# inai17ibar/video-diffusion-pipeline-parallel

Measured on AMD Instinct MI355X. Metric: steady-state videos/sec (whole node), SVD 14f x 25step, higher is better.
Workload: dtype f16

## Files before the change

### video-diffusion-pipeline-parallel_amd/csrc/gemm.hip

```cpp
#include <cstring>
#include "gemm_args.h"
#include <stdlib.h>

using namespace spgemm;

namespace {


template <int BM, int BN, int WM, int WN, int STAGES>
__global__ __launch_bounds__(WM *WN * 64, 2) void gemm_f16_kernel(const GemmArgs p) {
  constexpr int NW = WM * WN;
  constexpr int THREADS = NW * 64;
  constexpr int WTM = BM / WM, WTN = BN / WN;
  constexpr int TN = WTN / 16;
  constexpr int TM = WTM / 16;
  constexpr int A_BYTES = BM * BK * 2;
  constexpr int B_BYTES = BN * BK * 2;
  constexpr int STAGE = A_BYTES + B_BYTES;
  constexpr int A_LOADS = BM / 8 / NW;
  constexpr int B_LOADS = BN / 8 / NW;
  constexpr int L = A_LOADS + B_LOADS;
  static_assert(A_LOADS * 8 * NW == BM && B_LOADS * 8 * NW == BN, "tile rows must split evenly over waves");
  static_assert(STAGES == 2 || STAGES == 3, "2- or 3-deep ring");
  extern __shared__ __attribute__((aligned(16))) char smem[];
// ... 505 lines not shown
    const int bms[2] = {256, 192}, bns[2] = {256, 320};
    for (int bi = 0; bi < 2; ++bi)
      for (int ni = 0; ni < 2; ++ni) {
        if ((bns[ni] == 256 && !ok256) || (bns[ni] == 320 && !ok320)) continue;
        const int blocks = ((d->m + bms[bi] - 1) / bms[bi]) * (d->n / bns[ni]);
        double score = (double)blocks / (((blocks + 255) / 256) * 256.0);
        if (bms[bi] == 192) score -= 0.06;
        if (bns[ni] == 320) score -= 0.01;
        if (score > best) { best = score; bm = bms[bi]; bn = bns[ni]; }
      }
    if (route == 2) {
      if ((g_route_bn == 256 && ok256) || (g_route_bn == 320 && ok320)) bn = g_route_bn;
      if (g_route_bm == 192 || g_route_bm == 256 || (g_route_bm == 128 && bn == 256)) bm = g_route_bm;
    }
    return launch_pp(a, bm, bn, s);
  }
  if (n128 && d->m >= 4096) return launch<256, 128, 4, 2, 3>(a, s);
  if (n128) return launch<128, 128, 2, 2, 2>(a, s);
  if (d->n % 160 == 0) return launch<128, 160, 2, 2, 2>(a, s);
  return launch<128, 64, 2, 2, 2>(a, s);
}

}

namespace spgemm {
static thread_local char g_last_kernel[96] = "";
void note_kernel(const char *fmt, ...) {
  va_list ap;
  va_start(ap, fmt);
  vsnprintf(g_last_kernel, sizeof(g_last_kernel), fmt, ap);
  va_end(ap);
}
void note_kernel_suffix(const char *suffix) {
  const size_t have = strlen(g_last_kernel);
  snprintf(g_last_kernel + have, sizeof(g_last_kernel) - have, "%s", suffix);
}
}

extern "C" const char *sp_gemm_last_kernel(void) { return spgemm::g_last_kernel; }

extern "C" size_t sp_gemm_workspace_bytes(const sp_gemm_desc *d) {
  if (!d || d->m <= 0 || d->n <= 0 || d->cin <= 0) return 0;
  const int taps = d->mode == SP_A_CONV3X3 ? 9 : d->mode == SP_A_TEMPORAL3 ? 3 : 1;
  int sk = splitk_slices(d, taps, false);
  const int forced = splitk_slices(d, taps, true);
  if (forced > sk) sk = forced;
  size_t need = (size_t)sk * d->m * d->n * sizeof(float);
  const int ltiles = d->n % 320 == 0 ? d->n / 320 : d->n / 256;
  const size_t ln_part = (d->ln_out && ltiles > 1) ? (size_t)d->m * ltiles * 2 * sizeof(float) : 0;
  return need > ln_part ? need : ln_part;
}

extern "C" int sp_gemm_set_route(int route, int bm, int bn) {
  SP_REQUIRE(route >= 0 && route <= 4,
             "sp_gemm_set_route: route %d (0 auto, 1 small tiles, 2 ping-pong, 3 persistent-stream, 4 split-K)", route);
  SP_REQUIRE(bm == 0 || bm == 128 || bm == 192 || bm == 256, "sp_gemm_set_route: bm %d", bm);
  SP_REQUIRE(bn == 0 || bn == 256 || bn == 320 || bn == 192, "sp_gemm_set_route: bn %d", bn);
  g_route = route; g_route_bm = bm; g_route_bn = bn;
  return SP_OK;
}

extern "C" int sp_gemm_f32out_f16(const void *a_, int64_t lda, const void *w, void *d, int m, int n, int k,
                                  const void *zero_page, void *stream) {
  SP_REQUIRE(a_ && w && d && zero_page, "sp_gemm_f32out_f16: null a/w/d/zero_page");
  SP_REQUIRE(m > 0 && n > 0 && n % 256 == 0, "sp_gemm_f32out_f16: n=%d must be a positive multiple of 256 (m=%d)", n, m);
  SP_REQUIRE(k >= 64 && k % 64 == 0, "sp_gemm_f32out_f16: k=%d must be a multiple of 64", k);
  SP_REQUIRE(lda >= k && lda % 8 == 0, "sp_gemm_f32out_f16: lda=%lld invalid", (long long)lda);
  SP_REQUIRE(((uintptr_t)d & 15) == 0, "sp_gemm_f32out_f16: d must be 16-byte aligned");
  GemmArgs a{};
  a.a = (const f16 *)a_; a.w = (const f16 *)w; a.zero = (const char *)zero_page;
  a.lda = lda; a.mode = SP_A_LINEAR; a.cin = k; a.taps = 1; a.m = m; a.n = n; a.k = k;
  a.oscale = 1.0f; a.bias2_rows = m; a.ldb2 = n;
  a.ksplit = 1; a.partial = (float *)d;
  return spgemm::launch_pp(a, 256, 256, (hipStream_t)stream);
}

extern "C" int sp_gemm_f16(const sp_gemm_desc *d, void *stream) {
  SP_REQUIRE(d != nullptr, "sp_gemm_f16: null descriptor");
  SP_REQUIRE(d->a && d->w && d->d && d->zero_page, "sp_gemm_f16: null a/w/d/zero_page");
  SP_REQUIRE(d->m > 0 && d->n > 0, "sp_gemm_f16: m,n must be positive (m=%d n=%d)", d->m, d->n);
  SP_REQUIRE(d->cin > 0 && d->cin % 64 == 0, "sp_gemm_f16: cin=%d must be a multiple of 64", d->cin);
  SP_REQUIRE(d->n % 64 == 0, "sp_gemm_f16: n=%d must be a multiple of 64", d->n);
  SP_REQUIRE(d->mode >= SP_A_LINEAR && d->mode <= SP_A_TEMPORAL3, "sp_gemm_f16: bad mode %d", d->mode);
  SP_REQUIRE(d->lda >= d->cin && d->lda % 8 == 0, "sp_gemm_f16: lda=%lld invalid", (long long)d->lda);
  SP_REQUIRE(d->ldd % 8 == 0 || d->n_store > 0, "sp_gemm_f16: ldd must be a multiple of 8");
  GemmArgs a{};
#ifdef SP_GEMM_EXPERIMENTS
  { const char *e = getenv("SP_GEMM_DBG"); a.dbg = e ? atoi(e) : 0; }
  { const char *e = getenv("SP_GEMM_STAGGER"); a.stagger = e ? atoi(e) : 0; }
#endif
  a.a = (const f16 *)d->a; a.w = (const f16 *)d->w; a.bias = d->bias; a.bias2 = d->bias2;
  a.res1 = (const f16 *)d->res1; a.res2 = (const f16 *)d->res2; a.d = (f16 *)d->d;
  a.ln_stats = d->ln_stats; a.ln_colsum = d->ln_colsum;
  a.ln_out = d->ln_out; a.ln_out_eps = d->ln_out_eps;
  a.gn_part = nullptr;
  if (d->gn_part) {
    SP_REQUIRE(!d->geglu && !d->ln_stats && !d->ln_out && !d->euler_out && d->n_store == 0 &&
                   d->m % 256 == 0 && (d->n % 256 == 0 || d->n % 320 == 0) && ((uintptr_t)d->gn_part & 15) == 0,
               "sp_gemm_f16: gn_part needs whole 256-row tiles (m = %d), n a multiple of 256 or 320 (n = %d), no geglu / "
               "folded LayerNorm / ln_out / n_store / Euler tail, and a 16-byte aligned buffer", d->m, d->n);
    a.gn_part = d->gn_part;
  }
  a.w_group_rows = 0; a.w_group_stride = 0;
  if (d->w_group_rows != 0) {
    SP_REQUIRE(d->w_group_rows > 0 && d->w_group_rows % 128 == 0 && d->w_group_stride > 0 && d->w_group_stride % 8 == 0 &&
                   d->mode == SP_A_LINEAR && !d->geglu && !d->euler_out && (d->n % 256 == 0 || d->n % 320 == 0) &&
                   !d->ln_stats && !d->ln_colsum,
               "sp_gemm_f16: per-row-group weights need SP_A_LINEAR, no geglu / Euler tail / folded LayerNorm (ln_stats), n a "
               "multiple of 256 or 320, w_group_rows a positive multiple of 128 (got %lld) and w_group_stride a positive multiple "
               "of 8 (got %lld)", (long long)d->w_group_rows, (long long)d->w_group_stride);
    a.w_group_rows = d->w_group_rows; a.w_group_stride = d->w_group_stride;
// ... 78 lines not shown
```

### video-diffusion-pipeline-parallel_amd/csrc/gemm_args.h

```cpp
#pragma once
#include "common.h"

namespace spgemm {

constexpr int BK = 64;

template <int N>
__device__ __forceinline__ void wait_vm_lgkm() {
  asm volatile("s_waitcnt vmcnt(%0) lgkmcnt(0)" ::"n"(N) : "memory");
}

struct GemmArgs {
  const f16 *a;
  const f16 *a2;
  int64_t lda2;
  int cin2;
  const f16 *w;
  const float *bias;
  const float *bias2;
  const f16 *res1;
  const f16 *res2;
  const f16 *eul_lat; f16 *eul_out; const f16 *eul_u; const float *eul_gs;
  int64_t eul_ldu, eul_hw;
  int eul_frames;
  float eul_c_out, eul_c_skip, eul_inv_sigma, eul_dt;
  const float *ln_stats;
  const float *ln_colsum;
  float *ln_out;
  float ln_out_eps;
  float *gn_part;
  float *ln_part;
  f16 *d;
  const char *zero;
  int64_t lda, ldr1, ldr2, ldd, hw, bias2_rows, ldb2;
  int64_t w_group_rows, w_group_stride;
  int mode, cin, taps;
  int n_img, hin, win, hout, wout, stride, ups;
  int frames;
  int m, n, k;
  float oscale, r1scale, r2scale;
  int geglu, n_store;
  int tiles_m, tiles_n;
  int ksplit;
  float *partial;
  int dbg;
  int stagger;
};

__device__ __forceinline__ int xcd_remap(int bid, int nwg) {
  const int q = nwg >> 3, r = nwg & 7;
  const int xcd = bid & 7;
  const int base = xcd < r ? xcd * (q + 1) : r * (q + 1) + (xcd - r) * q;
  return base + (bid >> 3);
}


void note_kernel(const char *fmt, ...);
void note_kernel_suffix(const char *suffix);

int launch_pp(GemmArgs &a, int bm, int bn, hipStream_t s);

bool ps_supported(const GemmArgs &a, int bm, int bn);
int launch_ps(GemmArgs &a, int bm, int bn, hipStream_t s);

}
```

### video-diffusion-pipeline-parallel_amd/csrc/gemm_pp.hip

```cpp
#include "gemm_args.h"
#include <stdlib.h>
#include <type_traits>

namespace spgemm {
namespace {

constexpr int PBK = 32, PNW = 8;


#ifdef SP_GEMM_EXPERIMENTS
constexpr int PP_TRACE_WGS = 16384, PP_TRACE_SLOTS = 12;
__device__ long long g_pp_trace[PP_TRACE_WGS * PP_TRACE_SLOTS];
#define PP_TRACE(slot)                                                                              \
  do {                                                                                              \
    if (threadIdx.x == 0 && blockIdx.x < PP_TRACE_WGS)                                              \
      g_pp_trace[blockIdx.x * PP_TRACE_SLOTS + (slot)] = wall_clock64();                            \
  } while (0)
#define PP_TRACE_CLK(slot)                                                                          \
  do {                                                                                              \
    if (threadIdx.x == 0 && blockIdx.x < PP_TRACE_WGS)                                              \
      g_pp_trace[blockIdx.x * PP_TRACE_SLOTS + (slot)] = (long long)__builtin_amdgcn_s_memtime();   \
  } while (0)
#else
#define PP_TRACE(slot) do {} while (0)
#define PP_TRACE_CLK(slot) do {} while (0)
#endif

__device__ __forceinline__ int swz4(int row) { return (0x78 >> (((row >> 2) & 3) * 2)) & 3; }

#ifndef SP_PP_STAGES_192_256
#define SP_PP_STAGES_192_256 4
#endif
constexpr int pp_stages(int bm, int bn) { return bm == 128 ? 3 : (bm == 192 && bn == 256 ? SP_PP_STAGES_192_256 : 4); }

template <int N>
__device__ __forceinline__ void wait_vm() { asm volatile("s_waitcnt vmcnt(%0)" ::"n"(N) : "memory"); }

template <int L>
__device__ __forceinline__ void wait_dma(int ksteps_left) {
  if (ksteps_left >= 3) wait_vm<3 * L>();
  else if (ksteps_left == 2) wait_vm<2 * L>();
  else if (ksteps_left == 1) wait_vm<L>();
  else wait_vm<0>();
}

#define WROWS_OF(pbm, wtm) ((pbm) / (wtm))
template <int PBM, int BN, int TN, int TM, int WTN, int WTM, bool GEGLU, int NT, bool GNRES = false>
__device__ __forceinline__ void pp_epilogue(const GemmArgs &p, f32x4 (&acc)[TN][TM], char *smem, int tile_m,
                                            int tile_n, int wm, int wn, int tid, int fr, int fq) {
  constexpr int bno = GEGLU ? BN / 2 : BN;
  constexpr int cpr = bno >> 3;
  constexpr int TNO = GEGLU ? TN / 2 : TN;
  constexpr int NCH = PBM * cpr, ITERS = (NCH + NT - 1) / NT, ITERS_A = ITERS / 2;
  static_assert(cpr % 8 == 0, "chunk swizzle works on aligned groups of 8 chunks");
  const int ncols_total = GEGLU ? p.n / 2 : p.n;
  const int nstore = p.n_store > 0 ? p.n_store : ncols_total;
  const int64_t mbase = (int64_t)tile_m * PBM;

  auto res_src = [&](const f16 *res, int64_t ldr, int it) -> const f16 * {
    const int idx = tid + it * NT;
    const int r = idx / cpr, c = idx - r * cpr;
    const int64_t m = mbase + r;
    const int col = tile_n * bno + c * 8;
    const bool ok = idx < NCH && m < p.m && col + 8 <= nstore;
    return ok ? res + m * ldr + col : (const f16 *)p.zero;
  };

  if (p.ln_stats) {
    f32x2 st[TM];
    const __amdgpu_buffer_rsrc_t s_rsrc = __builtin_amdgcn_make_buffer_rsrc(
        (void *)p.ln_stats, 0, (int)min((int64_t)p.m * 8, (int64_t)0x7fffffff), 0x00020000);
#pragma unroll
    for (int j = 0; j < TM; ++j)
      st[j] = __builtin_bit_cast(f32x2, __builtin_amdgcn_raw_buffer_load_b64(
          s_rsrc, (int)((mbase + wm * WTM + j * 16 + fr) * 8), 0, 0));
#pragma unroll
    for (int i = 0; i < TN; ++i) {
      const int n = tile_n * BN + wn * WTN + i * 16 + 4 * fq;
      const f32x4 cs = *(const f32x4 *)(p.ln_colsum + n);
      f32x4 b = {0.f, 0.f, 0.f, 0.f};
      if (p.bias) b = *(const f32x4 *)(p.bias + n);
#pragma unroll
      for (int j = 0; j < TM; ++j) acc[i][j] = (acc[i][j] - st[j][0] * cs) * st[j][1] + b;
      __builtin_amdgcn_sched_barrier(0);
    }
  }
  if constexpr (!GEGLU) {
    if (p.gn_part && !p.res1 && !p.res2) {
      auto row16_sum = [](float v) {
        v += __builtin_bit_cast(float, __builtin_amdgcn_mov_dpp(__builtin_bit_cast(int, v), 0xB1, 0xF, 0xF, true));
        v += __builtin_bit_cast(float, __builtin_amdgcn_mov_dpp(__builtin_bit_cast(int, v), 0x4E, 0xF, 0xF, true));
        v += __builtin_bit_cast(float, __builtin_amdgcn_mov_dpp(__builtin_bit_cast(int, v), 0x141, 0xF, 0xF, true));
        v += __builtin_bit_cast(float, __builtin_amdgcn_mov_dpp(__builtin_bit_cast(int, v), 0x140, 0xF, 0xF, true));
        return v;
      };
      float *dst = p.gn_part + (((int64_t)tile_m * WROWS_OF(PBM, WTM) + wm) * p.n + (int64_t)tile_n * BN + wn * WTN) * 2;
#pragma unroll
      for (int i = 0; i < TN; ++i) {
        f32x4 sm = {0.f, 0.f, 0.f, 0.f}, sq = {0.f, 0.f, 0.f, 0.f};
#pragma unroll
        for (int j = 0; j < TM; ++j) {
          const f32x4 v = acc[i][j] * p.oscale;
          sm += v;
          sq += v * v;
        }
#pragma unroll
        for (int r = 0; r < 4; ++r) { sm[r] = row16_sum(sm[r]); sq[r] = row16_sum(sq[r]); }
        if (fr == 0) {
          float *o = dst + (i * 16 + 4 * fq) * 2;
          *(f32x4 *)o = (f32x4){sm[0], sq[0], sm[1], sq[1]};
          *(f32x4 *)(o + 4) = (f32x4){sm[2], sq[2], sm[3], sq[3]};
        }
      }
    }
  }
  f16x8 q1[ITERS];
  if (p.res1) {
#pragma unroll
    for (int it = 0; it < ITERS_A; ++it) q1[it] = *(const f16x8 *)res_src(p.res1, p.ldr1, it);
  }
  PP_TRACE(4);

#pragma unroll
  for (int i = 0; i < TNO; ++i) {
    const int col = (GEGLU ? (wn * WTN) / 2 : wn * WTN) + i * 16 + 4 * fq;
#pragma unroll
    for (int j = 0; j < TM; ++j) {
      f16x4 o;
      if constexpr (!GEGLU) {
        const f32x4 v = acc[i][j] * p.oscale;
        o = (f16x4){(f16)v[0], (f16)v[1], (f16)v[2], (f16)v[3]};
      } else {
        const f32x4 h = acc[2 * i][j] * p.oscale, g = acc[2 * i + 1][j];
        const f32x2 ga = gelu2_f((f32x2){g[0], g[1]}), gb = gelu2_f((f32x2){g[2], g[3]});
        o = (f16x4){(f16)(h[0] * ga[0]), (f16)(h[1] * ga[1]), (f16)(h[2] * gb[0]), (f16)(h[3] * gb[1])};
      }
      const int row = wm * WTM + j * 16 + fr;
      *(f16x4 *)(smem + row * (bno * 2) + ((((col >> 3) ^ (fr & 7))) << 4) + (col & 4) * 2) = o;
    }
  }
  if (p.res1) {
#pragma unroll
    for (int it = ITERS_A; it < ITERS; ++it) q1[it] = *(const f16x8 *)res_src(p.res1, p.ldr1, it);
  }
  asm volatile("s_waitcnt lgkmcnt(0)\n\ts_barrier" ::: "memory");
  PP_TRACE(6);

  f16x8 o[ITERS];
#pragma unroll
  for (int it = 0; it < ITERS; ++it) {
    const int idx = tid + it * NT;
    const int r = idx / cpr, c = idx - r * cpr;
    o[it] = *(const f16x8 *)(smem + r * (bno * 2) + ((c ^ (r & 7)) << 4));
  }
  const bool gn_res = GNRES && !GEGLU && PBM == 256 && p.gn_part && (p.res1 || p.res2);
  if (gn_res) asm volatile("s_waitcnt lgkmcnt(0)\n\ts_barrier" ::: "memory");
  if (p.res1 || p.res2) {
// ... 107 lines not shown
#pragma unroll
        for (int e = 0; e < 4; ++e) { pt[(grp * Q + quad) * 8 + 2 * e] = sm[e]; pt[(grp * Q + quad) * 8 + 2 * e + 1] = sq[e]; }
      }
      asm volatile("s_waitcnt lgkmcnt(0)\n\ts_barrier" ::: "memory");
      if (tid < 2 * Q) {
        const int half = tid / Q, qd = tid - half * Q;
        f32x4 a = {0.f, 0.f, 0.f, 0.f}, b = {0.f, 0.f, 0.f, 0.f};
        for (int sub = 0; sub < RG; ++sub) {
          const float *src = pt + ((half * RG + sub) * Q + qd) * 8;
          a += *(const f32x4 *)src; b += *(const f32x4 *)(src + 4);
        }
        float *dst = p.gn_part + (((int64_t)tile_m * 2 + half) * p.n + (int64_t)tile_n * bno + qd * 4) * 2;
        *(f32x4 *)dst = a;
        *(f32x4 *)(dst + 4) = b;
      }
    }
  }
}

#ifdef SP_GEMM_EXPERIMENTS
template <int TN, int TM, int NAP, int NBP, int NWV>
__device__ __forceinline__ void mfma_block(f32x4 (&acc)[TN][TM], const f16x8 (&fw)[TN], const f16x8 (&fa)[TM],
                                           const f16 *(&aptr)[NAP], int (&astep)[NAP], const f16 *(&bptr)[NBP],
                                           char *dsa, char *dsb, int pieces) {
  constexpr int NP = NAP + NBP, NM = TN * TM, GAP = NM / (NP + 1);
#pragma unroll
  for (int i = 0; i < TN; ++i) {
#pragma unroll
    for (int j = 0; j < TM; ++j) {
      acc[i][j] = __builtin_amdgcn_mfma_f32_16x16x32_f16(fw[i], fa[j], acc[i][j], 0, 0, 0);
      const int q1 = i * TM + j + 1;
      if (q1 % GAP == 0 && q1 / GAP <= NP) {
        const int pc = q1 / GAP - 1;
        if (pieces & (1 << pc)) {
          if (pc < NAP) {
            glds16(aptr[pc], dsa + pc * (NWV * 1024));
            aptr[pc] += astep[pc];
          } else {
            glds16(bptr[pc - NAP], dsb + (pc - NAP) * (NWV * 1024));
            bptr[pc - NAP] += PBK;
          }
        }
      }
    }
  }
}
#endif

template <int BM, int BN, int EXP>
__global__ __launch_bounds__(BM == 128 ? 256 : 512, 2) void gemm_pp_kernel(const GemmArgs p) {
  constexpr int PBM = BM;
  constexpr bool SPLITK = (EXP & 128) != 0;
  constexpr bool A2 = (EXP & 4096) != 0;
  constexpr int NWV = BM == 128 ? 4 : 8, NT = NWV * 64, WROWS = NWV / 4;
  constexpr int PSTAGES = pp_stages(BM, BN), PDIST = PSTAGES - 1;
  constexpr int TN = BN / 4 / 16;
  constexpr int TM = BM / WROWS / 16;
  constexpr int WTN = BN / 4, WTM = BM / WROWS;
  constexpr int A_BYTES = PBM * 64, B_BYTES = BN * 64, STAGE = A_BYTES + B_BYTES;
  constexpr int A_PIECES = BM / 16, B_PIECES = BN / 16;
  constexpr int A_LOADS = (A_PIECES + NWV - 1) / NWV, A_LOADS_HI = A_PIECES / NWV;
  constexpr int A_SPLIT = A_PIECES % NWV == 0 ? NWV : A_PIECES % NWV;
  constexpr int B_LOADS_LO = (B_PIECES + NWV - 1) / NWV;
  constexpr int B_LOADS_HI = B_PIECES / NWV;
  constexpr int B_SPLIT = B_PIECES % NWV == 0 ? NWV : B_PIECES % NWV;
  static_assert((B_SPLIT == NWV || B_SPLIT == 4) && (A_SPLIT == NWV || A_SPLIT == 4), "wave halves must have uniform DMA counts");
#ifdef SP_GEMM_EXPERIMENTS
  constexpr bool HALO_COUNT = (EXP & 16) != 0;
  constexpr int L_EARLY = (HALO_COUNT ? 0 : A_LOADS) + B_LOADS_LO;
  constexpr int L_LATE = (HALO_COUNT ? 0 : (A_SPLIT == NWV ? A_LOADS : A_LOADS_HI)) + (B_SPLIT == NWV ? B_LOADS_LO : B_LOADS_HI);
#else
  constexpr int L_EARLY = A_LOADS + B_LOADS_LO;
  constexpr int L_LATE = (A_SPLIT == NWV ? A_LOADS : A_LOADS_HI) + (B_SPLIT == NWV ? B_LOADS_LO : B_LOADS_HI);
#endif
  extern __shared__ __attribute__((aligned(16))) char smem[];

  const int tid = threadIdx.x, lane = tid & 63;
  const int wave = __builtin_amdgcn_readfirstlane(tid >> 6);
  const int wm = wave >> 2, wn = wave & 3;
  const bool late = NWV == 8 && wave >= 4;
#ifdef SP_GEMM_EXPERIMENTS
  if (p.stagger > 0 && blockIdx.x < 256) {
    const int d = ((blockIdx.x >> 3) & 3) * p.stagger;
    for (int i = 0; i < d; ++i) __builtin_amdgcn_s_sleep(30);
  }
#endif
  PP_TRACE(0);
#ifdef SP_GEMM_EXPERIMENTS
  if (tid == 0 && blockIdx.x < PP_TRACE_WGS) {
    const unsigned hw = __builtin_amdgcn_s_getreg((31 << 11) | 4);
    const unsigned xcc = __builtin_amdgcn_s_getreg((31 << 11) | 20);
    g_pp_trace[blockIdx.x * PP_TRACE_SLOTS + 5] = ((long long)xcc << 32) | hw;
  }
#endif

  constexpr int GM = BM == 128 ? 8 : 4;
  const int nwg = p.tiles_m * p.tiles_n;
  int bid = blockIdx.x, kslice = 0;
  if constexpr (SPLITK) { kslice = bid / nwg; bid -= kslice * nwg; }
  const int t = xcd_remap(bid, nwg);
  const int per_group = GM * p.tiles_n;
  const int group = t / per_group;
  const int first_m = group * GM;
  const int gsz = min(p.tiles_m - first_m, GM);
  const int in_group = t - group * per_group;
  const int tile_n = in_group / gsz;
// ... 76 lines not shown
  };

  const f16 *bptr[B_LOADS_LO];
#pragma unroll
  for (int j = 0; j < B_LOADS_LO; ++j) {
    const int piece = j * NWV + wave;
    const int r = piece * 16 + lrow;
    const int n = tile_n * BN + (r < BN ? r : 0);
    bptr[j] = p.w + (int64_t)n * p.k + (lchunk ^ swz4(r)) * 8;
    if (p.w_group_rows > 0) bptr[j] += ((int64_t)tile_m * PBM / p.w_group_rows) * p.w_group_stride;
  }

  bool skip_a = false;
  auto stage = [&](int slot) {
    char *sa = smem + slot * STAGE;
    char *sb = sa + A_BYTES;
#pragma unroll
    for (int i = 0; i < A_LOADS; ++i) {
      if ((i < A_LOADS_HI || wave < A_SPLIT) && !skip_a) {
        glds16(aptr[i], sa + (i * NWV + wave) * 1024);
        aptr[i] += astep[i];
      }
    }
#pragma unroll
    for (int j = 0; j < B_LOADS_LO; ++j) {
      if (j < B_LOADS_HI || wave < B_SPLIT) {
        glds16(bptr[j], sb + (j * NWV + wave) * 1024);
        bptr[j] += PBK;
      }
    }
  };

  f32x4 acc[TN][TM], bias_v[TN];
#pragma unroll
  for (int i = 0; i < TN; ++i) {
    bias_v[i] = (f32x4){0.f, 0.f, 0.f, 0.f};
    if (p.bias && !p.ln_stats && !SPLITK)
      bias_v[i] = *(const f32x4 *)(p.bias + tile_n * BN + wn * WTN + i * 16 + 4 * (lane >> 4));
  }
  __builtin_amdgcn_sched_barrier(0);

  int nk = p.k >> 5, kbeg = 0;
  if constexpr (SPLITK) {
    kbeg = (int)((int64_t)kslice * nk / p.ksplit);
    nk = (int)((int64_t)(kslice + 1) * nk / p.ksplit) - kbeg;
  }
  const int fr = lane & 15, fq = lane >> 4;
  const int rd_chunk = (fq ^ swz4(fr)) << 4;
  int offw[TN], offa[TM];
#pragma unroll
  for (int i = 0; i < TN; ++i) offw[i] = (wn * WTN + i * 16 + fr) * 64 + rd_chunk;
#pragma unroll
  for (int j = 0; j < TM; ++j) offa[j] = (wm * WTM + j * 16 + fr) * 64 + rd_chunk;

  int staged = 0, in_tap = 0, tap = 0, stage_slot = 0, read_slot = 0;
  auto stage_next = [&]() {
    if (in_tap == cpt && (!A2 || tap < p.taps)) { ++tap; in_tap = 0; set_tap(tap); }
#ifdef SP_GEMM_EXPERIMENTS
    if constexpr ((EXP & 16) != 0) skip_a = tap > 0;
#endif
    stage(stage_slot);
    stage_slot = stage_slot + 1 == PSTAGES ? 0 : stage_slot + 1;
    ++staged; ++in_tap;
  };
  tap = kbeg / cpt;
  in_tap = kbeg - tap * cpt;
  set_tap(tap);
  if (kbeg) {
#pragma unroll
    for (int i = 0; i < A_LOADS; ++i) aptr[i] += in_tap * astep[i];
#pragma unroll
    for (int j = 0; j < B_LOADS_LO; ++j) bptr[j] += (int64_t)kbeg * PBK;
  }
  PP_TRACE(10);
#pragma unroll
  for (int s = 0; s < PDIST; ++s)
    if (s < nk) stage_next();
  PP_TRACE(11);
  __builtin_amdgcn_sched_barrier(0);
  if (p.bias2 && !SPLITK) {
    int brow[TM];
#pragma unroll
    for (int j = 0; j < TM; ++j) {
      const int m = tile_m * PBM + wm * WTM + j * 16 + fr;
      brow[j] = m < p.m ? m / (int)p.bias2_rows : 0;
    }
#pragma unroll
    for (int i = 0; i < TN; ++i) {
      const int n = tile_n * BN + wn * WTN + i * 16 + 4 * fq;
#pragma unroll
      for (int j = 0; j < TM; ++j) acc[i][j] = *(const f32x4 *)(p.bias2 + (int64_t)brow[j] * p.ldb2 + n) + bias_v[i];
      __builtin_amdgcn_sched_barrier(0);
    }
  } else {
#pragma unroll
    for (int i = 0; i < TN; ++i)
#pragma unroll
      for (int j = 0; j < TM; ++j) acc[i][j] = bias_v[i];
  }
  {
    const int left = min(PDIST - 1, nk - 1);
    if (late) wait_dma<L_LATE>(left); else wait_dma<L_EARLY>(left);
  }
  __builtin_amdgcn_s_barrier();
  if (late) __builtin_amdgcn_s_barrier();
  PP_TRACE(1);
  PP_TRACE_CLK(8);

#ifdef SP_GEMM_EXPERIMENTS
  constexpr int dbg = EXP;
  constexpr bool DMA_IN_COMPUTE = (dbg & 4) != 0;
#endif
  for (int kt = 0; kt < nk; ++kt) {
    const bool issue = kt + PDIST < nk;
    const char *sa = smem + read_slot * STAGE;
    read_slot = read_slot + 1 == PSTAGES ? 0 : read_slot + 1;
    const char *sb = sa + A_BYTES;
    f16x8 fw[TN], fa[TM];
#ifdef SP_GEMM_EXPERIMENTS
    if ((dbg & 64) && kt > 0) {
#pragma unroll
      for (int i = 0; i < TN; ++i) fw[i] = (f16x8){1, 2, 3, 4, 5, 6, 7, (f16)kt};
#pragma unroll
      for (int j = 0; j < TM; ++j) fa[j] = (f16x8){1, 2, 3, 4, 5, 6, 7, (f16)lane};
    } else
#endif
    {
#pragma unroll
      for (int i = 0; i < TN; ++i) fw[i] = *(const f16x8 *)(sb + offw[i]);
#pragma unroll
      for (int j = 0; j < TM; ++j) fa[j] = *(const f16x8 *)(sa + offa[j]);
    }
#ifdef SP_GEMM_EXPERIMENTS
    if constexpr ((dbg & 32) != 0) {
      const f16x2 sc2 = {(f16)(1.0f + 0.001f * lane), (f16)1.0f}, sh2 = {(f16)0.01f, (f16)(0.002f * lane)};
#pragma unroll
      for (int j = 0; j < TM; ++j) {
#pragma unroll
        for (int e = 0; e < 4; ++e) {
          f16x2 v = {fa[j][2 * e], fa[j][2 * e + 1]};
          v = __builtin_elementwise_fma(v, sc2, sh2);
          const f16x2 t = __builtin_elementwise_exp2(v * (f16x2){(f16)-1.4427f, (f16)-1.4427f}) + (f16x2){(f16)1.0f, (f16)1.0f};
          v = v * (f16x2){(f16)__builtin_amdgcn_rcph(t[0]), (f16)__builtin_amdgcn_rcph(t[1])};
          fa[j][2 * e] = v[0]; fa[j][2 * e + 1] = v[1];
        }
      }
    }
#endif
    __builtin_amdgcn_sched_barrier(0);
#ifdef SP_GEMM_EXPERIMENTS
    if constexpr (DMA_IN_COMPUTE) {
      if (issue && in_tap == cpt) { ++tap; in_tap = 0; set_tap(tap); }
      int left = min(PDIST - 2, nk - 2 - kt);
      if (left < 0) left = 0;
      if (late) wait_dma<L_LATE>(left);
    } else
#endif
    {
#ifdef SP_GEMM_EXPERIMENTS
      if constexpr (!(dbg & 1))
#endif
      { if (issue) stage_next(); }
      int left = min(PDIST - 1, nk - 2 - kt);
      if (left < 0) left = 0;
      if (late) wait_dma<L_LATE>(left);
    }
    asm volatile("s_waitcnt lgkmcnt(0)" ::: "memory");
    __builtin_amdgcn_sched_barrier(0);
    __builtin_amdgcn_s_barrier();
    __builtin_amdgcn_sched_barrier(0);
    __builtin_amdgcn_s_setprio(1);
#ifdef SP_GEMM_EXPERIMENTS
    if constexpr (DMA_IN_COMPUTE) {
      char *dsa = smem + stage_slot * STAGE + wave * 1024;
      char *dsb = dsa + A_BYTES;
      int pieces = 0;
      if (issue) {
#pragma unroll
        for (int i = 0; i < A_LOADS; ++i) if (i < A_LOADS_HI || wave < A_SPLIT) pieces |= 1 << i;
#pragma unroll
        for (int j = 0; j < B_LOADS_LO; ++j) if (j < B_LOADS_HI || wave < B_SPLIT) pieces |= 1 << (A_LOADS + j);
      }
      mfma_block<TN, TM, A_LOADS, B_LOADS_LO, NWV>(acc, fw, fa, aptr, astep, bptr, dsa, dsb,
                                              __builtin_amdgcn_readfirstlane(pieces));
      if (issue) {
        stage_slot = stage_slot + 1 == PSTAGES ? 0 : stage_slot + 1;
        ++staged; ++in_tap;
      }
    } else if constexpr ((dbg & 2) != 0) {
#pragma unroll
      for (int i = 0; i < TN; ++i) asm volatile("" ::"v"(fw[i]));
#pragma unroll
      for (int j = 0; j < TM; ++j) asm volatile("" ::"v"(fa[j]));
    } else
#endif
    {
#pragma unroll
      for (int i = 0; i < TN; ++i) {
#pragma unroll
        for (int j = 0; j < TM; ++j)
          acc[i][j] = __builtin_amdgcn_mfma_f32_16x16x32_f16(fw[i], fa[j], acc[i][j], 0, 0, 0);
      }
    }
    __builtin_amdgcn_s_setprio(0);
    if (!late) wait_dma<L_EARLY>(min(PDIST - 1, max(nk - 2 - kt, 0)));
    __builtin_amdgcn_sched_barrier(0);
    __builtin_amdgcn_s_barrier();
    __builtin_amdgcn_sched_barrier(0);
  }
  if (!late) __builtin_amdgcn_s_barrier();
  PP_TRACE_CLK(9);
  PP_TRACE(2);

  if constexpr (SPLITK) {
    float *slab = p.partial + (int64_t)kslice * p.m * p.n;
#pragma unroll
    for (int j = 0; j < TM; ++j) {
      const int64_t m = (int64_t)tile_m * PBM + wm * WTM + j * 16 + fr;
      if (m < p.m) {
#pragma unroll
        for (int i = 0; i < TN; ++i)
          *(f32x4 *)(slab + m * p.n + tile_n * BN + wn * WTN + i * 16 + 4 * fq) = acc[i][j];
      }
    }
  } else if (p.geglu) {
    if constexpr (TN % 2 == 0) pp_epilogue<PBM, BN, TN, TM, WTN, WTM, true, NT>(p, acc, smem, tile_m, tile_n, wm, wn, tid, fr, fq);
  } else {
    pp_epilogue<PBM, BN, TN, TM, WTN, WTM, false, NT, (EXP & 2048) != 0>(p, acc, smem, tile_m, tile_n, wm, wn, tid, fr, fq);
  }
  PP_TRACE(3);
}

template <int BM, int BN, int EXP = 0>
int launch_pp(GemmArgs &a, hipStream_t s) {
  constexpr int NSTG = pp_stages(BM, BN);
  constexpr size_t ring = (size_t)NSTG * (BM + BN) * 64, tile = (size_t)BM * BN * 2;
  constexpr size_t lds = ring > tile ? ring : tile;
  static_assert(lds <= 160 * 1024, "LDS per workgroup");
  static bool attr_set[SP_MAX_DEVICES] = {};
  if (int rc = sp_ensure_dyn_lds((const void *)gemm_pp_kernel<BM, BN, EXP>, (int)lds, attr_set, "sp_gemm_f16(pp)"))
    return rc;
  a.tiles_m = (a.m + BM - 1) / BM;
  a.tiles_n = a.n / BN;
  note_kernel((EXP & 128) ? "gemm_pp_kernel<%d, %d, %d> + splitk_reduce_kernel" : "gemm_pp_kernel<%d, %d, %d>", BM, BN, EXP);
  SP_CLEAR_STALE_ERROR();
  hipLaunchKernelGGL((gemm_pp_kernel<BM, BN, EXP>), dim3(a.tiles_m * a.tiles_n * ((EXP & 128) ? a.ksplit : 1)),
                     dim3(BM == 128 ? 256 : 512), lds, s, a);
  SP_CHECK_LAUNCH("sp_gemm_f16(pp)");
  return SP_OK;
}

}

int launch_pp(GemmArgs &a, int bm, int bn, hipStream_t s) {
  if (a.ksplit >= 1 && a.partial) return launch_pp<256, 256, 128>(a, s);
  if (a.gn_part && (a.res1 || a.res2)) return bn == 256 ? launch_pp<256, 256, 2048>(a, s) : launch_pp<256, 320, 2048>(a, s);
  if (a.a2) return bn == 256 ? launch_pp<256, 256, 4096>(a, s) : launch_pp<256, 320, 4096>(a, s);
#ifdef SP_GEMM_EXPERIMENTS
  if (bm == 256 && bn == 256) switch (a.dbg) {
    case 1: return launch_pp<256, 256, 1>(a, s);
    case 2: return launch_pp<256, 256, 2>(a, s);
    case 3: return launch_pp<256, 256, 3>(a, s);
    case 65: return launch_pp<256, 256, 65>(a, s);
    case 67: return launch_pp<256, 256, 67>(a, s);
    case 4: return launch_pp<256, 256, 4>(a, s);
    default: break;
  }
  if (bm == 256 && bn == 320 && a.dbg == 4) return launch_pp<256, 320, 4>(a, s);
  if (bm == 192 && bn == 256 && a.dbg == 4) return launch_pp<192, 256, 4>(a, s);
  if (a.dbg == 16) {
    if (bm == 256 && bn == 256) return launch_pp<256, 256, 16>(a, s);
    if (bm == 256 && bn == 320) return launch_pp<256, 320, 16>(a, s);
    if (bm == 192 && bn == 256) return launch_pp<192, 256, 16>(a, s);
  }
  if (a.dbg == 32 && bm == 256 && bn == 320) return launch_pp<256, 320, 32>(a, s);
  if (a.dbg == 8) {
    if (bm == 256 && bn == 256) return launch_pp<256, 256, 8>(a, s);
    if (bm == 256 && bn == 320) return launch_pp<256, 320, 8>(a, s);
    if (bm == 192 && bn == 256) return launch_pp<192, 256, 8>(a, s);
  }
#endif
  if (bn == 256) {
    if (bm == 128) return launch_pp<128, 256>(a, s);
    if (bm == 192) return launch_pp<192, 256>(a, s);
    return launch_pp<256, 256>(a, s);
  }
  if (bm == 192) return launch_pp<192, 320>(a, s);
  return launch_pp<256, 320>(a, s);
}

}

#ifdef SP_GEMM_EXPERIMENTS
extern "C" int sp_debug_pp_trace(long long *host, int n_wgs) {
  if (n_wgs > spgemm::PP_TRACE_WGS) n_wgs = spgemm::PP_TRACE_WGS;
  return (int)hipMemcpyFromSymbol(host, HIP_SYMBOL(spgemm::g_pp_trace),
                                  sizeof(long long) * n_wgs * spgemm::PP_TRACE_SLOTS);
}
#endif
```

Baseline: 0.8151.

## Add whole-line paired K-step staging path to ping-pong GEMM

Adds a new ping-pong GEMM mainloop variant that stages two 32-wide K steps at once as full 128-byte lines per row, loaded directly into LDS via buffer/global load-to-LDS instructions, into a two-image double buffer. Out-of-range rows are handled with buffer out-of-bounds offsets instead of zero-page pointers. The variant becomes the default for 256-row tiles when alignment and size checks pass, and a route flag can force the old ring. The aim is wider, better-coalesced loads with fewer barriers and waits per K step. The cost is less pipelining depth (two images instead of a 4-stage ring) and more complex addressing. It also switches the GN sum of squares to explicit fma.

```diff
diff --git a/video-diffusion-pipeline-parallel_amd/csrc/gemm.hip b/video-diffusion-pipeline-parallel_amd/csrc/gemm.hip
--- a/video-diffusion-pipeline-parallel_amd/csrc/gemm.hip
+++ b/video-diffusion-pipeline-parallel_amd/csrc/gemm.hip
@@ -581,11 +581,13 @@
 }
 
 extern "C" int sp_gemm_set_route(int route, int bm, int bn) {
-  SP_REQUIRE(route >= 0 && route <= 4,
-             "sp_gemm_set_route: route %d (0 auto, 1 small tiles, 2 ping-pong, 3 persistent-stream, 4 split-K)", route);
+  SP_REQUIRE(route >= 0 && (route & 15) <= 4 && (route >> 4) <= 2,
+             "sp_gemm_set_route: route %d (0 auto, 1 small tiles, 2 ping-pong, 3 persistent-stream, 4 split-K; "
+             "+16 ping-pong K-step ring only, +32 ping-pong whole-line pairs wherever supported)", route);
   SP_REQUIRE(bm == 0 || bm == 128 || bm == 192 || bm == 256, "sp_gemm_set_route: bm %d", bm);
   SP_REQUIRE(bn == 0 || bn == 256 || bn == 320 || bn == 192, "sp_gemm_set_route: bn %d", bn);
-  g_route = route; g_route_bm = bm; g_route_bn = bn;
+  g_route = route & 15; g_route_bm = bm; g_route_bn = bn;
+  spgemm::g_pp_lines = route >> 4;
   return SP_OK;
 }
 
diff --git a/video-diffusion-pipeline-parallel_amd/csrc/gemm_args.h b/video-diffusion-pipeline-parallel_amd/csrc/gemm_args.h
--- a/video-diffusion-pipeline-parallel_amd/csrc/gemm_args.h
+++ b/video-diffusion-pipeline-parallel_amd/csrc/gemm_args.h
@@ -59,6 +59,7 @@
 void note_kernel_suffix(const char *suffix);
 
 int launch_pp(GemmArgs &a, int bm, int bn, hipStream_t s);
+extern int g_pp_lines;
 
 bool ps_supported(const GemmArgs &a, int bm, int bn);
 int launch_ps(GemmArgs &a, int bm, int bn, hipStream_t s);
diff --git a/video-diffusion-pipeline-parallel_amd/csrc/gemm_pp.hip b/video-diffusion-pipeline-parallel_amd/csrc/gemm_pp.hip
--- a/video-diffusion-pipeline-parallel_amd/csrc/gemm_pp.hip
+++ b/video-diffusion-pipeline-parallel_amd/csrc/gemm_pp.hip
@@ -44,6 +44,23 @@
   else wait_vm<0>();
 }
 
+__device__ __forceinline__ void glds16_s(const char *sbase, unsigned voff, char *lds_dst) {
+  const unsigned l = (unsigned)(uintptr_t)(__attribute__((address_space(3))) char *)lds_dst;
+  asm volatile("s_mov_b32 m0, %2\n\ts_nop 0\n\tglobal_load_lds_dwordx4 %0, %1"
+               :: "v"(voff), "s"(sbase), "s"(l) : "memory", "m0");
+}
+typedef unsigned v4u_t __attribute__((__vector_size__(4 * sizeof(unsigned))));
+constexpr unsigned BUF_OOB = 0x80000000u;
+__device__ __forceinline__ v4u_t buf_rsrc(const void *base) {
+  const uint64_t b = (uint64_t)(uintptr_t)base;
+  return (v4u_t){(unsigned)b, (unsigned)(b >> 32) & 0xffffu, 0x7fffffffu, 0x00020000u};
+}
+__device__ __forceinline__ void blds16(v4u_t rsrc, unsigned voff, unsigned soff, char *lds_dst) {
+  const unsigned l = (unsigned)(uintptr_t)(__attribute__((address_space(3))) char *)lds_dst;
+  asm volatile("s_mov_b32 m0, %3\n\ts_nop 0\n\tbuffer_load_dwordx4 %0, %1, %2 offen lds"
+               :: "v"(voff), "s"(rsrc), "s"(soff), "s"(l) : "memory", "m0");
+}
+
 #define WROWS_OF(pbm, wtm) ((pbm) / (wtm))
 template <int PBM, int BN, int TN, int TM, int WTN, int WTM, bool GEGLU, int NT, bool GNRES = false>
 __device__ __forceinline__ void pp_epilogue(const GemmArgs &p, f32x4 (&acc)[TN][TM], char *smem, int tile_m,
@@ -102,7 +119,8 @@
         for (int j = 0; j < TM; ++j) {
           const f32x4 v = acc[i][j] * p.oscale;
           sm += v;
-          sq += v * v;
+#pragma unroll
+          for (int r = 0; r < 4; ++r) sq[r] = __builtin_fmaf(v[r], v[r], sq[r]);
         }
 #pragma unroll
         for (int r = 0; r < 4; ++r) { sm[r] = row16_sum(sm[r]); sq[r] = row16_sum(sq[r]); }
@@ -316,6 +334,7 @@
   constexpr int PBM = BM;
   constexpr bool SPLITK = (EXP & 128) != 0;
   constexpr bool A2 = (EXP & 4096) != 0;
+  constexpr bool WL = (EXP & 8192) != 0;
   constexpr int NWV = BM == 128 ? 4 : 8, NT = NWV * 64, WROWS = NWV / 4;
   constexpr int PSTAGES = pp_stages(BM, BN), PDIST = PSTAGES - 1;
   constexpr int TN = BN / 4 / 16;
@@ -498,163 +517,295 @@
   for (int i = 0; i < TN; ++i) offw[i] = (wn * WTN + i * 16 + fr) * 64 + rd_chunk;
 #pragma unroll
   for (int j = 0; j < TM; ++j) offa[j] = (wm * WTM + j * 16 + fr) * 64 + rd_chunk;
-
-  int staged = 0, in_tap = 0, tap = 0, stage_slot = 0, read_slot = 0;
-  auto stage_next = [&]() {
-    if (in_tap == cpt && (!A2 || tap < p.taps)) { ++tap; in_tap = 0; set_tap(tap); }
-#ifdef SP_GEMM_EXPERIMENTS
-    if constexpr ((EXP & 16) != 0) skip_a = tap > 0;
-#endif
-    stage(stage_slot);
-    stage_slot = stage_slot + 1 == PSTAGES ? 0 : stage_slot + 1;
-    ++staged; ++in_tap;
+  auto init_acc = [&]() {
+    if (p.bias2 && !SPLITK) {
+      int brow[TM];
+#pragma unroll
+      for (int j = 0; j < TM; ++j) {
+        const int m = tile_m * PBM + wm * WTM + j * 16 + fr;
+        brow[j] = m < p.m ? m / (int)p.bias2_rows : 0;
+      }
+#pragma unroll
+      for (int i = 0; i < TN; ++i) {
+        const int n = tile_n * BN + wn * WTN + i * 16 + 4 * fq;
+#pragma unroll
+        for (int j = 0; j < TM; ++j) acc[i][j] = *(const f32x4 *)(p.bias2 + (int64_t)brow[j] * p.ldb2 + n) + bias_v[i];
+        __builtin_amdgcn_sched_barrier(0);
+      }
+    } else {
+#pragma unroll
+      for (int i = 0; i < TN; ++i)
+#pragma unroll
+        for (int j = 0; j < TM; ++j) acc[i][j] = bias_v[i];
+    }
   };
-  tap = kbeg / cpt;
-  in_tap = kbeg - tap * cpt;
-  set_tap(tap);
-  if (kbeg) {
-#pragma unroll
-    for (int i = 0; i < A_LOADS; ++i) aptr[i] += in_tap * astep[i];
-#pragma unroll
-    for (int j = 0; j < B_LOADS_LO; ++j) bptr[j] += (int64_t)kbeg * PBK;
-  }
-  PP_TRACE(10);
-#pragma unroll
-  for (int s = 0; s < PDIST; ++s)
-    if (s < nk) stage_next();
-  PP_TRACE(11);
-  __builtin_amdgcn_sched_barrier(0);
-  if (p.bias2 && !SPLITK) {
-    int brow[TM];
-#pragma unroll
-    for (int j = 0; j < TM; ++j) {
-      const int m = tile_m * PBM + wm * WTM + j * 16 + fr;
-      brow[j] = m < p.m ? m / (int)p.bias2_rows : 0;
-    }
-#pragma unroll
-    for (int i = 0; i < TN; ++i) {
-      const int n = tile_n * BN + wn * WTN + i * 16 + 4 * fq;
-#pragma unroll
-      for (int j = 0; j < TM; ++j) acc[i][j] = *(const f32x4 *)(p.bias2 + (int64_t)brow[j] * p.ldb2 + n) + bias_v[i];
-      __builtin_amdgcn_sched_barrier(0);
-    }
+
+  if constexpr (!WL) {
+    int staged = 0, in_tap = 0, tap = 0, stage_slot = 0, read_slot = 0;
+    auto stage_next = [&]() {
+      if (in_tap == cpt && (!A2 || tap < p.taps)) { ++tap; in_tap = 0; set_tap(tap); }
+#ifdef SP_GEMM_EXPERIMENTS
+      if constexpr ((EXP & 16) != 0) skip_a = tap > 0;
+#endif
+      stage(stage_slot);
+      stage_slot = stage_slot + 1 == PSTAGES ? 0 : stage_slot + 1;
+      ++staged; ++in_tap;
+    };
+    tap = kbeg / cpt;
+    in_tap = kbeg - tap * cpt;
+    set_tap(tap);
+    if (kbeg) {
+#pragma unroll
+      for (int i = 0; i < A_LOADS; ++i) aptr[i] += in_tap * astep[i];
+#pragma unroll
+      for (int j = 0; j < B_LOADS_LO; ++j) bptr[j] += (int64_t)kbeg * PBK;
+    }
+    PP_TRACE(10);
+#pragma unroll
+    for (int s = 0; s < PDIST; ++s)
+      if (s < nk) stage_next();
+    PP_TRACE(11);
+    __builtin_amdgcn_sched_barrier(0);
+    init_acc();
+    {
+      const int left = min(PDIST - 1, nk - 1);
+      if (late) wait_dma<L_LATE>(left); else wait_dma<L_EARLY>(left);
+    }
+    __builtin_amdgcn_s_barrier();
+    if (late) __builtin_amdgcn_s_barrier();
+    PP_TRACE(1);
+    PP_TRACE_CLK(8);
+
+#ifdef SP_GEMM_EXPERIMENTS
+    constexpr int dbg = EXP;
+    constexpr bool DMA_IN_COMPUTE = (dbg & 4) != 0;
+#endif
+    for (int kt = 0; kt < nk; ++kt) {
+      const bool issue = kt + PDIST < nk;
+      const char *sa = smem + read_slot * STAGE;
+      read_slot = read_slot + 1 == PSTAGES ? 0 : read_slot + 1;
+      const char *sb = sa + A_BYTES;
+      f16x8 fw[TN], fa[TM];
+#ifdef SP_GEMM_EXPERIMENTS
+      if ((dbg & 64) && kt > 0) {
+#pragma unroll
+        for (int i = 0; i < TN; ++i) fw[i] = (f16x8){1, 2, 3, 4, 5, 6, 7, (f16)kt};
+#pragma unroll
+        for (int j = 0; j < TM; ++j) fa[j] = (f16x8){1, 2, 3, 4, 5, 6, 7, (f16)lane};
+      } else
+#endif
+      {
+#pragma unroll
+        for (int i = 0; i < TN; ++i) fw[i] = *(const f16x8 *)(sb + offw[i]);
+#pragma unroll
+        for (int j = 0; j < TM; ++j) fa[j] = *(const f16x8 *)(sa + offa[j]);
+      }
+#ifdef SP_GEMM_EXPERIMENTS
+      if constexpr ((dbg & 32) != 0) {
+        const f16x2 sc2 = {(f16)(1.0f + 0.001f * lane), (f16)1.0f}, sh2 = {(f16)0.01f, (f16)(0.002f * lane)};
+#pragma unroll
+        for (int j = 0; j < TM; ++j) {
+#pragma unroll
+          for (int e = 0; e < 4; ++e) {
+            f16x2 v = {fa[j][2 * e], fa[j][2 * e + 1]};
+            v = __builtin_elementwise_fma(v, sc2, sh2);
+            const f16x2 t = __builtin_elementwise_exp2(v * (f16x2){(f16)-1.4427f, (f16)-1.4427f}) + (f16x2){(f16)1.0f, (f16)1.0f};
+            v = v * (f16x2){(f16)__builtin_amdgcn_rcph(t[0]), (f16)__builtin_amdgcn_rcph(t[1])};
+            fa[j][2 * e] = v[0]; fa[j][2 * e + 1] = v[1];
+          }
+        }
+      }
+#endif
+      __builtin_amdgcn_sched_barrier(0);
+#ifdef SP_GEMM_EXPERIMENTS
+      if constexpr (DMA_IN_COMPUTE) {
+        if (issue && in_tap == cpt) { ++tap; in_tap = 0; set_tap(tap); }
+        int left = min(PDIST - 2, nk - 2 - kt);
+        if (left < 0) left = 0;
+        if (late) wait_dma<L_LATE>(left);
+      } else
+#endif
+      {
+#ifdef SP_GEMM_EXPERIMENTS
+        if constexpr (!(dbg & 1))
+#endif
+        { if (issue) stage_next(); }
+        int left = min(PDIST - 1, nk - 2 - kt);
+        if (left < 0) left = 0;
+        if (late) wait_dma<L_LATE>(left);
+      }
+      asm volatile("s_waitcnt lgkmcnt(0)" ::: "memory");
+      __builtin_amdgcn_sched_barrier(0);
+      __builtin_amdgcn_s_barrier();
+      __builtin_amdgcn_sched_barrier(0);
+      __builtin_amdgcn_s_setprio(1);
+#ifdef SP_GEMM_EXPERIMENTS
+      if constexpr (DMA_IN_COMPUTE) {
+        char *dsa = smem + stage_slot * STAGE + wave * 1024;
+        char *dsb = dsa + A_BYTES;
+        int pieces = 0;
+        if (issue) {
+#pragma unroll
+          for (int i = 0; i < A_LOADS; ++i) if (i < A_LOADS_HI || wave < A_SPLIT) pieces |= 1 << i;
+#pragma unroll
+          for (int j = 0; j < B_LOADS_LO; ++j) if (j < B_LOADS_HI || wave < B_SPLIT) pieces |= 1 << (A_LOADS + j);
+        }
+        mfma_block<TN, TM, A_LOADS, B_LOADS_LO, NWV>(acc, fw, fa, aptr, astep, bptr, dsa, dsb,
+                                                __builtin_amdgcn_readfirstlane(pieces));
+        if (issue) {
+          stage_slot = stage_slot + 1 == PSTAGES ? 0 : stage_slot + 1;
+          ++staged; ++in_tap;
+        }
+      } else if constexpr ((dbg & 2) != 0) {
+#pragma unroll
+        for (int i = 0; i < TN; ++i) asm volatile("" ::"v"(fw[i]));
+#pragma unroll
+        for (int j = 0; j < TM; ++j) asm volatile("" ::"v"(fa[j]));
+      } else
+#endif
+      {
+#pragma unroll
+        for (int i = 0; i < TN; ++i) {
+#pragma unroll
+          for (int j = 0; j < TM; ++j)
+            acc[i][j] = __builtin_amdgcn_mfma_f32_16x16x32_f16(fw[i], fa[j], acc[i][j], 0, 0, 0);
+        }
+      }
+      __builtin_amdgcn_s_setprio(0);
+      if (!late) wait_dma<L_EARLY>(min(PDIST - 1, max(nk - 2 - kt, 0)));
+      __builtin_amdgcn_sched_barrier(0);
+      __builtin_amdgcn_s_barrier();
+      __builtin_amdgcn_sched_barrier(0);
+    }
+    if (!late) __builtin_amdgcn_s_barrier();
   } else {
-#pragma unroll
-    for (int i = 0; i < TN; ++i)
-#pragma unroll
-      for (int j = 0; j < TM; ++j) acc[i][j] = bias_v[i];
-  }
-  {
-    const int left = min(PDIST - 1, nk - 1);
-    if (late) wait_dma<L_LATE>(left); else wait_dma<L_EARLY>(left);
-  }
-  __builtin_amdgcn_s_barrier();
-  if (late) __builtin_amdgcn_s_barrier();
-  PP_TRACE(1);
-  PP_TRACE_CLK(8);
-
-#ifdef SP_GEMM_EXPERIMENTS
-  constexpr int dbg = EXP;
-  constexpr bool DMA_IN_COMPUTE = (dbg & 4) != 0;
-#endif
-  for (int kt = 0; kt < nk; ++kt) {
-    const bool issue = kt + PDIST < nk;
-    const char *sa = smem + read_slot * STAGE;
-    read_slot = read_slot + 1 == PSTAGES ? 0 : read_slot + 1;
-    const char *sb = sa + A_BYTES;
-    f16x8 fw[TN], fa[TM];
-#ifdef SP_GEMM_EXPERIMENTS
-    if ((dbg & 64) && kt > 0) {
-#pragma unroll
-      for (int i = 0; i < TN; ++i) fw[i] = (f16x8){1, 2, 3, 4, 5, 6, 7, (f16)kt};
-#pragma unroll
-      for (int j = 0; j < TM; ++j) fa[j] = (f16x8){1, 2, 3, 4, 5, 6, 7, (f16)lane};
-    } else
-#endif
-    {
-#pragma unroll
-      for (int i = 0; i < TN; ++i) fw[i] = *(const f16x8 *)(sb + offw[i]);
-#pragma unroll
-      for (int j = 0; j < TM; ++j) fa[j] = *(const f16x8 *)(sa + offa[j]);
-    }
-#ifdef SP_GEMM_EXPERIMENTS
-    if constexpr ((dbg & 32) != 0) {
-      const f16x2 sc2 = {(f16)(1.0f + 0.001f * lane), (f16)1.0f}, sh2 = {(f16)0.01f, (f16)(0.002f * lane)};
-#pragma unroll
-      for (int j = 0; j < TM; ++j) {
-#pragma unroll
-        for (int e = 0; e < 4; ++e) {
-          f16x2 v = {fa[j][2 * e], fa[j][2 * e + 1]};
-          v = __builtin_elementwise_fma(v, sc2, sh2);
-          const f16x2 t = __builtin_elementwise_exp2(v * (f16x2){(f16)-1.4427f, (f16)-1.4427f}) + (f16x2){(f16)1.0f, (f16)1.0f};
-          v = v * (f16x2){(f16)__builtin_amdgcn_rcph(t[0]), (f16)__builtin_amdgcn_rcph(t[1])};
-          fa[j][2 * e] = v[0]; fa[j][2 * e + 1] = v[1];
-        }
-      }
-    }
-#endif
+    constexpr int AW = BM / 64, BW = BN / 64;
+    constexpr int LW = AW + BW;
+    constexpr int IMG = (BM + BN) * 128, B_OFF = BM * 128;
+    static_assert(BM == 256 && NWV == 8, "whole-line pairs: 256-row tiles of 8 waves");
+    const int frow = lane >> 3;
+    const unsigned fchunk = (unsigned)(((lane & 7) ^ frow) * 16);
+    constexpr int FAR = -(1 << 20);
+    int g0[AW], g1[AW], g2[AW];
+#pragma unroll
+    for (int i = 0; i < AW; ++i) {
+      const int m = tile_m * PBM + (i * 8 + wave) * 8 + frow;
+      const bool in = m < p.m;
+      if (p.mode == SP_A_CONV3X3) {
+        const int per_img = p.hout * p.wout;
+        const int img = m / per_img, rem = m - img * per_img, oy = rem / p.wout;
+        g0[i] = img;
+        g1[i] = in ? oy * p.stride - 1 : FAR;
+        g2[i] = (rem - oy * p.wout) * p.stride - 1;
+      } else if (p.mode == SP_A_TEMPORAL3) {
+        g0[i] = in ? (m / (int)p.hw) % p.frames : FAR;
+        g1[i] = 0;
+        g2[i] = m;
+      } else {
+        g0[i] = g1[i] = 0;
+        g2[i] = in ? m : -1;
+      }
+    }
+    unsigned a_off[AW], a_k = 0;
+    v4u_t a_rsrc;
+    auto set_tap_w = [&](int tap) {
+      const bool extra = A2 && tap == p.taps;
+      a_rsrc = buf_rsrc(extra ? (const void *)p.a2 : (const void *)p.a);
+      const unsigned ldb = (unsigned)((extra ? p.lda2 : p.lda) * 2);
+#pragma unroll
+      for (int i = 0; i < AW; ++i) {
+        int row = -1;
+        if (extra) {
+          const int m = tile_m * PBM + (i * 8 + wave) * 8 + frow;
+          row = m < p.m ? m : -1;
+        } else if (p.mode == SP_A_CONV3X3) {
+          const int ky = tap / 3, kx = tap - ky * 3;
+          const int iy = g1[i] + ky, ix = g2[i] + kx;
+          const int hv = p.hin << p.ups, wv = p.win << p.ups;
+          if (iy >= 0 && iy < hv && ix >= 0 && ix < wv) row = (g0[i] * p.hin + (iy >> p.ups)) * p.win + (ix >> p.ups);
+        } else if (p.mode == SP_A_TEMPORAL3) {
+          const int f = g0[i] + tap - 1;
+          if (f >= 0 && f < p.frames) row = g2[i] + (tap - 1) * (int)p.hw;
+        } else {
+          row = g2[i];
+        }
+        a_off[i] = row >= 0 ? (unsigned)row * ldb + fchunk : BUF_OOB;
+      }
+      a_k = 0;
+    };
+    unsigned b_off[BW];
+#pragma unroll
+    for (int j = 0; j < BW; ++j) b_off[j] = (unsigned)(((j * 8 + wave) * 8 + frow) * p.k * 2) + fchunk;
+    const char *b_src = (const char *)(p.w + (int64_t)tile_n * BN * p.k);
+    if (p.w_group_rows > 0) b_src += ((int64_t)tile_m * PBM / p.w_group_rows) * p.w_group_stride * 2;
+
+    const int cpt = p.cin >> 5;
+    int tap = kbeg / cpt, in_tap = kbeg - tap * cpt;
+    set_tap_w(tap);
+    a_k = (unsigned)in_tap * 64;
+    b_src += (int64_t)kbeg * 64;
+    auto stage_w = [&](int img) {
+      if (in_tap == cpt && (!A2 || tap < p.taps)) { ++tap; in_tap = 0; set_tap_w(tap); }
+      char *sa = smem + img * IMG;
+#pragma unroll
+      for (int i = 0; i < AW; ++i) blds16(a_rsrc, a_off[i], a_k, sa + (i * 8 + wave) * 1024);
+#pragma unroll
+      for (int j = 0; j < BW; ++j) glds16_s(b_src, b_off[j], sa + B_OFF + (j * 8 + wave) * 1024);
+      a_k += 128;
+      b_src += 128;
+      in_tap += 2;
+    };
+
+    PP_TRACE(10);
+    stage_w(0);
+    if (nk > 2) stage_w(1);
+    PP_TRACE(11);
     __builtin_amdgcn_sched_barrier(0);
-#ifdef SP_GEMM_EXPERIMENTS
-    if constexpr (DMA_IN_COMPUTE) {
-      if (issue && in_tap == cpt) { ++tap; in_tap = 0; set_tap(tap); }
-      int left = min(PDIST - 2, nk - 2 - kt);
-      if (left < 0) left = 0;
-      if (late) wait_dma<L_LATE>(left);
-    } else
-#endif
-    {
-#ifdef SP_GEMM_EXPERIMENTS
-      if constexpr (!(dbg & 1))
-#endif
-      { if (issue) stage_next(); }
-      int left = min(PDIST - 1, nk - 2 - kt);
-      if (left < 0) left = 0;
-      if (late) wait_dma<L_LATE>(left);
-    }
-    asm volatile("s_waitcnt lgkmcnt(0)" ::: "memory");
-    __builtin_amdgcn_sched_barrier(0);
+    init_acc();
+    if (nk > 2) wait_vm<LW>(); else wait_vm<0>();
     __builtin_amdgcn_s_barrier();
-    __builtin_amdgcn_sched_barrier(0);
-    __builtin_amdgcn_s_setprio(1);
-#ifdef SP_GEMM_EXPERIMENTS
-    if constexpr (DMA_IN_COMPUTE) {
-      char *dsa = smem + stage_slot * STAGE + wave * 1024;
-      char *dsb = dsa + A_BYTES;
-      int pieces = 0;
-      if (issue) {
-#pragma unroll
-        for (int i = 0; i < A_LOADS; ++i) if (i < A_LOADS_HI || wave < A_SPLIT) pieces |= 1 << i;
-#pragma unroll
-        for (int j = 0; j < B_LOADS_LO; ++j) if (j < B_LOADS_HI || wave < B_SPLIT) pieces |= 1 << (A_LOADS + j);
-      }
-      mfma_block<TN, TM, A_LOADS, B_LOADS_LO, NWV>(acc, fw, fa, aptr, astep, bptr, dsa, dsb,
-                                              __builtin_amdgcn_readfirstlane(pieces));
-      if (issue) {
-        stage_slot = stage_slot + 1 == PSTAGES ? 0 : stage_slot + 1;
-        ++staged; ++in_tap;
-      }
-    } else if constexpr ((dbg & 2) != 0) {
-#pragma unroll
-      for (int i = 0; i < TN; ++i) asm volatile("" ::"v"(fw[i]));
-#pragma unroll
-      for (int j = 0; j < TM; ++j) asm volatile("" ::"v"(fa[j]));
-    } else
-#endif
-    {
+    if (late) __builtin_amdgcn_s_barrier();
+    PP_TRACE(1);
+    PP_TRACE_CLK(8);
+
+    const int rd = (fq ^ (fr & 7)) << 4;
+    const int offw0 = B_OFF + (wn * WTN + fr) * 128 + rd, offa0 = (wm * WTM + fr) * 128 + rd;
+    auto kstep = [&](int kt, auto odd_c) {
+      constexpr int ODD = decltype(odd_c)::value;
+      const char *sa = smem + ((kt >> 1) & 1) * IMG;
+      const int ow = offw0 ^ (ODD << 6), oa = offa0 ^ (ODD << 6);
+      f16x8 fw[TN], fa[TM];
+#pragma unroll
+      for (int i = 0; i < TN; ++i) fw[i] = *(const f16x8 *)(sa + ow + i * 16 * 128);
+#pragma unroll
+      for (int j = 0; j < TM; ++j) fa[j] = *(const f16x8 *)(sa + oa + j * 16 * 128);
+      __builtin_amdgcn_sched_barrier(0);
+      if (!ODD && kt >= 2 && kt + 2 < nk) stage_w(((kt >> 1) + 1) & 1);
+      const bool need = ODD && kt + 1 < nk;
+      if (late && need) wait_vm<0>();
+      asm volatile("s_waitcnt lgkmcnt(0)" ::: "memory");
+      __builtin_amdgcn_sched_barrier(0);
+      __builtin_amdgcn_s_barrier();
+      __builtin_amdgcn_sched_barrier(0);
+      __builtin_amdgcn_s_setprio(1);
 #pragma unroll
       for (int i = 0; i < TN; ++i) {
 #pragma unroll
         for (int j = 0; j < TM; ++j)
           acc[i][j] = __builtin_amdgcn_mfma_f32_16x16x32_f16(fw[i], fa[j], acc[i][j], 0, 0, 0);
       }
-    }
-    __builtin_amdgcn_s_setprio(0);
-    if (!late) wait_dma<L_EARLY>(min(PDIST - 1, max(nk - 2 - kt, 0)));
-    __builtin_amdgcn_sched_barrier(0);
-    __builtin_amdgcn_s_barrier();
-    __builtin_amdgcn_sched_barrier(0);
-  }
-  if (!late) __builtin_amdgcn_s_barrier();
+      __builtin_amdgcn_s_setprio(0);
+      if (!late && need) wait_vm<0>();
+      __builtin_amdgcn_sched_barrier(0);
+      __builtin_amdgcn_s_barrier();
+      __builtin_amdgcn_sched_barrier(0);
+    };
+    for (int kt = 0; kt < nk; kt += 2) {
+      kstep(kt, std::integral_constant<int, 0>{});
+      kstep(kt + 1, std::integral_constant<int, 1>{});
+    }
+    if (!late) __builtin_amdgcn_s_barrier();
+  }
   PP_TRACE_CLK(9);
   PP_TRACE(2);
 
@@ -696,12 +847,44 @@
   return SP_OK;
 }
 
-}
+bool wl_supported(const GemmArgs &a, int bm) {
+  if (bm != 256) return false;
+  if (a.cin % 64 || a.k % 64 || a.lda % 64 || ((uintptr_t)a.a & 127) || ((uintptr_t)a.w & 127)) return false;
+  if (a.a2 && (a.cin2 % 64 || a.lda2 % 64 || ((uintptr_t)a.a2 & 127))) return false;
+  const int64_t rows = a.mode == SP_A_CONV3X3 ? (int64_t)a.n_img * a.hin * a.win : (int64_t)a.m;
+  const int64_t lim = (int64_t)1 << 31;
+  if ((rows + 1) * a.lda * 2 >= lim || (a.a2 && ((int64_t)a.m + 1) * a.lda2 * 2 >= lim)) return false;
+  if ((int64_t)320 * a.k * 2 >= lim) return false;
+  if (a.ksplit >= 1 && a.partial) {
+    const int nk = a.k / 32;
+    for (int s = 1; s < a.ksplit; ++s)
+      if (((int64_t)s * nk / a.ksplit) & 1) return false;
+  }
+  return true;
+}
+
+}
+
+int g_pp_lines = 0;
 
 int launch_pp(GemmArgs &a, int bm, int bn, hipStream_t s) {
-  if (a.ksplit >= 1 && a.partial) return launch_pp<256, 256, 128>(a, s);
-  if (a.gn_part && (a.res1 || a.res2)) return bn == 256 ? launch_pp<256, 256, 2048>(a, s) : launch_pp<256, 320, 2048>(a, s);
-  if (a.a2) return bn == 256 ? launch_pp<256, 256, 4096>(a, s) : launch_pp<256, 320, 4096>(a, s);
+  const bool wl = wl_supported(a, bm) && g_pp_lines != 1;
+  if (a.ksplit >= 1 && a.partial)
+    return wl ? launch_pp<256, 256, 128 | 8192>(a, s) : launch_pp<256, 256, 128>(a, s);
+  if (a.gn_part && (a.res1 || a.res2)) {
+    if (wl) return bn == 256 ? launch_pp<256, 256, 2048 | 8192>(a, s) : launch_pp<256, 320, 2048 | 8192>(a, s);
+    return bn == 256 ? launch_pp<256, 256, 2048>(a, s) : launch_pp<256, 320, 2048>(a, s);
+  }
+  if (a.a2) {
+    if (wl) return bn == 256 ? launch_pp<256, 256, 4096 | 8192>(a, s) : launch_pp<256, 320, 4096 | 8192>(a, s);
+    return bn == 256 ? launch_pp<256, 256, 4096>(a, s) : launch_pp<256, 320, 4096>(a, s);
+  }
+  if (wl
+#ifdef SP_GEMM_EXPERIMENTS
+      && a.dbg == 0
+#endif
+  )
+    return bn == 256 ? launch_pp<256, 256, 8192>(a, s) : launch_pp<256, 320, 8192>(a, s);
 #ifdef SP_GEMM_EXPERIMENTS
   if (bm == 256 && bn == 256) switch (a.dbg) {
     case 1: return launch_pp<256, 256, 1>(a, s);
```

Result: faster. 0.8244 (median of 6 runs) (+1.1%).
